# brunnergino/MIDI-VAE

Hardware: AMD Instinct MI355X
Metric: MIDI roll windows/sec (train step) (higher is better)
Workload: dtype bf16

## Files before the change

### midi-vae_amd/csrc/latent.hip

```cpp
#include "common.h"

namespace {

constexpr int LR = 4;
constexpr int LT = 512;
constexpr float CE_EPS = 1e-7f;

template <bool TANH>
__device__ void dense_rows(const float* xs, int ldx, const float* __restrict__ W, int ldw, const float* __restrict__ bias,
                           int K, int N, float* red, float* ys, int ldy, float* yg, int ldg) {
    const int t = threadIdx.x, NV = N / 4;
    for (int c0 = 0; c0 < NV; c0 += LT) {
        const int cur = min(LT, NV - c0), KS = LT / cur, nvl = t % cur, ks = t / cur;
        const int per = ((K + KS - 1) / KS + 3) & ~3;
        if (ks < KS) {
            const int n = (c0 + nvl) * 4;
            f32x4 acc[LR];
#pragma unroll
            for (int r = 0; r < LR; ++r) acc[r] = f32x4{0.f, 0.f, 0.f, 0.f};
            const int k0 = ks * per, k1 = min(K, k0 + per);
            int k = k0;
            for (; k + 16 <= k1; k += 16) {
                f32x4 wv[16];
#pragma unroll
                for (int u = 0; u < 16; ++u) wv[u] = *reinterpret_cast<const f32x4*>(W + (size_t)(k + u) * ldw + n);
#pragma unroll
                for (int r = 0; r < LR; ++r)
#pragma unroll
                    for (int u = 0; u < 16; u += 4) {
                        const f32x4 x = *reinterpret_cast<const f32x4*>(xs + r * ldx + k + u);
                        acc[r] += x[0] * wv[u] + x[1] * wv[u + 1] + x[2] * wv[u + 2] + x[3] * wv[u + 3];
                    }
            }
            for (; k + 4 <= k1; k += 4) {
                f32x4 wv[4];
#pragma unroll
                for (int u = 0; u < 4; ++u) wv[u] = *reinterpret_cast<const f32x4*>(W + (size_t)(k + u) * ldw + n);
#pragma unroll
                for (int r = 0; r < LR; ++r) {
                    const f32x4 x = *reinterpret_cast<const f32x4*>(xs + r * ldx + k);
                    acc[r] += x[0] * wv[0] + x[1] * wv[1] + x[2] * wv[2] + x[3] * wv[3];
                }
            }
            for (; k < k1; ++k) {
                const f32x4 w0 = *reinterpret_cast<const f32x4*>(W + (size_t)k * ldw + n);
#pragma unroll
                for (int r = 0; r < LR; ++r) acc[r] += xs[r * ldx + k] * w0;
            }
#pragma unroll
            for (int r = 0; r < LR; ++r) *reinterpret_cast<f32x4*>(red + ((size_t)(ks * LR + r) * cur + nvl) * 4) = acc[r];
        }
        __syncthreads();
        for (int e = t; e < LR * cur; e += LT) {
            const int r = e / cur, c = e % cur, n = (c0 + c) * 4;
            f32x4 v = {0.f, 0.f, 0.f, 0.f};
            if (bias) v = f32x4{bias[n], bias[n + 1], bias[n + 2], bias[n + 3]};
            for (int s = 0; s < KS; ++s) v += *reinterpret_cast<const f32x4*>(red + ((size_t)(s * LR + r) * cur + c) * 4);
            if (TANH) v = f32x4{tanhf(v[0]), tanhf(v[1]), tanhf(v[2]), tanhf(v[3])};
            if (ys) *reinterpret_cast<f32x4*>(ys + r * ldy + n) = v;
            if (yg) *reinterpret_cast<f32x4*>(yg + (size_t)r * ldg + n) = v;
        }
        __syncthreads();
    }
}

__device__ __forceinline__ int pad4(int n) { return (n + 3) & ~3; }

__global__ __launch_bounds__(LT) void latent_chain_fwd_k(const mvae_latent_chain_fwd_args a) {
    extern __shared__ __attribute__((aligned(16))) float sm[];
    const int H = a.H, Z = a.Z, zin = a.zin, ncH = a.ncat * H, t = threadIdx.x;
    const int r0 = blockIdx.x * LR;
    float* xcat = sm;
    float* h1 = xcat + LR * pad4(ncH);
    float* h2 = h1 + LR * H;
    float* mu = h2 + LR * H;
    float* lv = mu + LR * pad4(Z);
    float* zh = lv + LR * pad4(Z);
    float* red = zh + LR * pad4(zin);
    for (int e = t; e < LR * ncH; e += LT) {
        const int r = e / ncH, c = e % ncH;
        xcat[r * pad4(ncH) + c] = a.cat[(size_t)(r0 + r) * ncH + c];
    }
    __syncthreads();
    const float* h = xcat;
    int ldh = pad4(ncH);
    if (a.w_pack) {
        dense_rows<true>(h, ldh, a.w_pack, H, a.b_pack, ncH, H, red, h1, H, a.pack + (size_t)r0 * H, H);
        h = h1;
        ldh = H;
    }
    if (a.w_extra) {
        dense_rows<true>(h, ldh, a.w_extra, H, a.b_extra, H, H, red, h2, H, a.extra + (size_t)r0 * H, H);
        h = h2;
        ldh = H;
    }
    const int h1w = a.split ? H / 2 : H, h2o = a.split ? h1w : 0, h2w = a.split ? H - h1w : H;
    dense_rows<false>(h, ldh, a.w_mu, Z, a.b_mu, h1w, Z, red, mu, pad4(Z), a.mu + (size_t)r0 * Z, Z);
    dense_rows<false>(h + h2o, ldh, a.w_lv, Z, a.b_lv, h2w, Z, red, lv, pad4(Z), a.logvar + (size_t)r0 * Z, Z);
    {
        const int w = t >> 6, l = t & 63;
        if (w < LR) {
            const int b = r0 + w;
            const float plv = 2.0f * logf(a.prior_std), pvar = a.prior_std * a.prior_std;
            float kl = 0.0f;
            for (int j = l; j < zin; j += 64) {
                float v;
                if (j < Z) {
                    const float m = mu[w * pad4(Z) + j], lg = lv[w * pad4(Z) + j];
                    const float d = m - a.prior_mean;
                    kl += 1.0f + lg - plv - (d * d + expf(lg)) / pvar;
                    v = m + expf(0.5f * lg) * a.eps[(size_t)b * Z + j];
                    a.zh[(size_t)b * zin + j] = v;
                } else {
                    v = a.zh[(size_t)b * zin + j];
                }
                zh[w * pad4(zin) + j] = v;
            }
            kl = wave_sum(kl);
            const bool styled = a.style_target && a.C > 0;
            if (l == 0 && b >= a.B_valid) {
                if (a.kl_rows) a.kl_rows[b] = 0.0f;
                if (a.style_rows && styled) {
                    a.style_rows[(size_t)b * 2] = 0.0f;
                    a.style_rows[(size_t)b * 2 + 1] = 0.0f;
                }
            }
            if (l == 0 && b < a.B_valid) {
                const float klb = a.inv_batch * a.beta * (-0.5f) * kl;
                atomicAdd(a.scalars, klb);
                if (a.kl_rows) a.kl_rows[b] = klb;
                if (styled) {
                    const int C = a.C;
                    const float* zr = zh + w * pad4(zin);
                    float mx = -INFINITY;
                    for (int c = 0; c < C; ++c) mx = fmaxf(mx, zr[c]);
                    float sum = 0.0f;
                    for (int c = 0; c < C; ++c) sum += expf(zr[c] - mx);
                    const int tg = a.style_target[b];
                    float pt = 0.0f, pm = -1.0f;
                    int am = 0;
                    for (int c = 0; c < C; ++c) {
                        const float p = expf(zr[c] - mx) / sum;
                        if (a.style_probs) a.style_probs[(size_t)b * C + c] = p;
                        if (c == tg) pt = p;
                        if (p > pm) { pm = p; am = c; }
                    }
                    const float rw = a.style_row_weight ? a.style_row_weight[b] : a.inv_batch;
                    const float ce = tg < C ? -logf(fminf(fmaxf(pt, CE_EPS), 1.0f - CE_EPS)) : 0.0f;
                    const float hit = am == (tg < C ? tg : 0) ? 1.0f : 0.0f;
                    atomicAdd(a.scalars + 1, rw * ce);
                    atomicAdd(a.scalars + 2, hit);
                    if (a.style_rows) {
                        a.style_rows[(size_t)b * 2] = rw * ce;
                        a.style_rows[(size_t)b * 2 + 1] = hit;
                    }
                }
            }
        }
        __syncthreads();
    }
    if (a.w_init)
        dense_rows<true>(zh, pad4(zin), a.w_init, a.n_init, a.b_init, zin, a.n_init, red, nullptr, 0,
                         a.S + (size_t)r0 * a.n_init, a.n_init);
}

__global__ __launch_bounds__(LT) void latent_chain_bwd_k(const mvae_latent_chain_bwd_args a) {
    extern __shared__ __attribute__((aligned(16))) float sm[];
    const int H = a.H, Z = a.Z, zin = a.zin, ncH = a.ncat * H, NI = a.n_init, t = threadIdx.x;
    const int r0 = blockIdx.x * LR;
    float* ds = sm;
    float* dzh = ds + LR * pad4(NI);
    float* dml = dzh + LR * pad4(zin);
    float* dt = dml + LR * 2 * pad4(Z);
    float* dt2 = dt + LR * H;
    float* dc = dt2 + LR * H;
    float* red = dc + LR * pad4(ncH);
    for (int e = t; e < LR * NI; e += LT) {
        const int r = e / NI, c = e % NI;
        const size_t g = (size_t)(r0 + r) * NI + c;
        const float s = a.S[g], v = a.dS[g] * (1.0f - s * s);
        a.dS[g] = v;
        ds[r * pad4(NI) + c] = v;
    }
    __syncthreads();
    dense_rows<false>(ds, pad4(NI), a.wt_init, zin, nullptr, NI, zin, red, dzh, pad4(zin), nullptr, 0);
    {
        const float pvar = a.prior_std * a.prior_std;
        for (int e = t; e < LR * Z; e += LT) {
            const int r = e / Z, j = e % Z, b = r0 + r;
            float dmu = 0.0f, dlv = 0.0f;
            if (b < a.B_valid) {
                float dz = dzh[r * pad4(zin) + j];
                if (a.style_probs && a.style_target && j < a.C) {
                    const int tg = a.style_target[b];
                    if (tg < a.C) {
                        const float pt = a.style_probs[(size_t)b * a.C + tg];
                        if (pt >= CE_EPS && pt <= 1.0f - CE_EPS) {
                            const float rw = a.style_row_weight ? a.style_row_weight[b] : a.inv_batch;
                            dz += a.style_weight * rw * (a.style_probs[(size_t)b * a.C + j] - (j == tg ? 1.0f : 0.0f));
                        }
                    }
                }
                const float m = a.mu[(size_t)b * Z + j], lg = a.logvar[(size_t)b * Z + j];
                dmu = dz + a.beta * (m - a.prior_mean) / pvar * a.inv_batch;
                dlv = dz * a.eps[(size_t)b * Z + j] * 0.5f * expf(0.5f * lg) +
                      a.beta * (-0.5f) * (1.0f - expf(lg) / pvar) * a.inv_batch;
            }
            a.dmu[(size_t)b * Z + j] = dmu;
            a.dlogvar[(size_t)b * Z + j] = dlv;
            dml[r * 2 * pad4(Z) + j] = dmu;
            dml[r * 2 * pad4(Z) + pad4(Z) + j] = dlv;
        }
        for (int e = t; e < LR * zin; e += LT) a.dzh[(size_t)(r0 + e / zin) * zin + e % zin] = dzh[(e / zin) * pad4(zin) + e % zin];
        __syncthreads();
    }
    const int h1w = a.split ? H / 2 : H, h2w = a.split ? H - h1w : H;
    dense_rows<false>(dml, 2 * pad4(Z), a.wt_mu, h1w, nullptr, Z, h1w, red, dt, H, nullptr, 0);
    if (a.split) {
        dense_rows<false>(dml + pad4(Z), 2 * pad4(Z), a.wt_lv, h2w, nullptr, Z, h2w, red, dt + h1w, H, nullptr, 0);
    } else {
        dense_rows<false>(dml + pad4(Z), 2 * pad4(Z), a.wt_lv, H, nullptr, Z, H, red, dt2, H, nullptr, 0);
        for (int e = t; e < LR * H; e += LT) dt[e] += dt2[e];
        __syncthreads();
    }
    float* cur = dt;
    if (a.wt_extra) {
        for (int e = t; e < LR * H; e += LT) {
            const size_t g = (size_t)(r0 + e / H) * H + e % H;
            const float y = a.extra[g], v = dt[e] * (1.0f - y * y);
            dt[e] = v;
            a.d_extra[g] = v;
        }
        __syncthreads();
        dense_rows<false>(dt, H, a.wt_extra, H, nullptr, H, H, red, dt2, H, nullptr, 0);
        cur = dt2;
    }
    if (a.wt_pack) {
        for (int e = t; e < LR * H; e += LT) {
            const size_t g = (size_t)(r0 + e / H) * H + e % H;
            const float y = a.pack[g], v = cur[e] * (1.0f - y * y);
            cur[e] = v;
            a.d_pack[g] = v;
        }
        __syncthreads();
        dense_rows<false>(cur, H, a.wt_pack, ncH, nullptr, H, ncH, red, nullptr, 0, a.dcat + (size_t)r0 * ncH, ncH);
    } else {
        for (int e = t; e < LR * H; e += LT) a.dcat[(size_t)(r0 + e / H) * H + e % H] = cur[e];
    }
}

size_t fwd_lds(const mvae_latent_chain_fwd_args& a) {
    auto p4 = [](int n) { return (n + 3) & ~3; };
    return sizeof(float) * ((size_t)LR * (p4(a.ncat * a.H) + 2 * a.H + 2 * p4(a.Z) + p4(a.zin)) + (size_t)4 * LR * LT);
}
size_t bwd_lds(const mvae_latent_chain_bwd_args& a) {
    auto p4 = [](int n) { return (n + 3) & ~3; };
    return sizeof(float) * ((size_t)LR * (p4(a.n_init) + p4(a.zin) + 2 * p4(a.Z) + 2 * a.H + p4(a.ncat * a.H)) + (size_t)4 * LR * LT);
}

}

extern "C" int mvae_latent_chain_fwd(const mvae_latent_chain_fwd_args* a, void* stream) {
    if (!a || a->B <= 0 || (a->B % LR) || a->H <= 0 || (a->H % 8) || a->Z <= 0 || (a->Z % 4) || (a->zin % 4) || a->zin < a->Z ||
        a->ncat < 1 || !a->cat || !a->w_mu || !a->w_lv || !a->mu || !a->logvar || !a->eps || !a->zh || !a->scalars)
        return MVAE_E_ARG;
    if ((a->w_pack && !a->pack) || (a->w_extra && !a->extra) || (a->w_init && (!a->S || a->n_init <= 0))) return MVAE_E_ARG;
    if (!a->w_pack && a->ncat != 1) return MVAE_E_ARG;
    if (a->w_init && (a->n_init % 4)) return MVAE_E_ARG;
    if (a->style_target && (a->C <= 0 || a->C > 64 || a->C > a->Z)) return MVAE_E_ARG;
    const size_t lds = fwd_lds(*a);
    if (lds > 160 * 1024) return MVAE_E_UNSUPPORTED;
    return mvae_launch<latent_chain_fwd_k>(dim3(a->B / LR), dim3(LT), lds, reinterpret_cast<hipStream_t>(stream), *a);
}

extern "C" int mvae_latent_chain_bwd(const mvae_latent_chain_bwd_args* a, void* stream) {
    if (!a || a->B <= 0 || (a->B % LR) || a->H <= 0 || (a->H % 8) || a->Z <= 0 || (a->Z % 4) || (a->zin % 4) || a->zin < a->Z ||
        a->ncat < 1 || a->n_init <= 0 || (a->n_init % 4) || !a->S || !a->dS || !a->wt_init || !a->wt_mu || !a->wt_lv || !a->mu ||
        !a->logvar || !a->eps || !a->dzh || !a->dmu || !a->dlogvar || !a->dcat)
        return MVAE_E_ARG;
    if ((a->wt_pack && (!a->pack || !a->d_pack)) || (a->wt_extra && (!a->extra || !a->d_extra))) return MVAE_E_ARG;
    if (!a->wt_pack && a->ncat != 1) return MVAE_E_ARG;
    const size_t lds = bwd_lds(*a);
    if (lds > 160 * 1024) return MVAE_E_UNSUPPORTED;
    return mvae_launch<latent_chain_bwd_k>(dim3(a->B / LR), dim3(LT), lds, reinterpret_cast<hipStream_t>(stream), *a);
}
```

Before: 40180.

## Double-buffer weight loads and prefetch next stage's first tile across dense stages

Rewrites dense_rows as a software-pipelined loop with two 16-row register buffers, loading the next weight tile while FMAs run on the current one. The first tile of the following layer is prefetched before the reduction barrier, so the chain of dense layers in the latent forward and backward kernels overlaps weight fetch latency with compute and with reductions. Tail rows are handled by clamped loads in place of the scalar remainder loops. This costs extra registers (two 16-entry f32x4 buffers), which may reduce occupancy or cause spills, and adds more control logic per iteration.

```diff
diff --git a/midi-vae_amd/csrc/latent.hip b/midi-vae_amd/csrc/latent.hip
--- a/midi-vae_amd/csrc/latent.hip
+++ b/midi-vae_amd/csrc/latent.hip
@@ -6,59 +6,110 @@
 constexpr int LT = 512;
 constexpr float CE_EPS = 1e-7f;
 
+struct Stage {
+    const float* W;
+    int ldw, K, N;
+};
+
+struct Slice {
+    int cur, KS, nvl, ks, n, k0, k1;
+};
+
+__device__ __forceinline__ Slice slice_of(const Stage& s, int c0) {
+    const int t = threadIdx.x, NV = s.N / 4;
+    Slice q;
+    q.cur = min(LT, NV - c0);
+    q.KS = LT / q.cur;
+    q.nvl = t % q.cur;
+    q.ks = t / q.cur;
+    const int per = ((s.K + q.KS - 1) / q.KS + 3) & ~3;
+    q.n = (c0 + q.nvl) * 4;
+    q.k0 = q.ks < q.KS ? q.ks * per : 0;
+    q.k1 = q.ks < q.KS ? min(s.K, q.k0 + per) : 0;
+    return q;
+}
+
+__device__ __forceinline__ void load_round(f32x4 (&b)[16], const float* __restrict__ W, int ldw, int K, int row0, int n) {
+    if (row0 + 16 <= K) {
+#pragma unroll
+        for (int u = 0; u < 16; ++u) b[u] = *reinterpret_cast<const f32x4*>(W + (size_t)(row0 + u) * ldw + n);
+    } else {
+#pragma unroll
+        for (int u = 0; u < 16; ++u) b[u] = *reinterpret_cast<const f32x4*>(W + (size_t)min(row0 + u, K - 1) * ldw + n);
+    }
+}
+
+__device__ __forceinline__ void prefetch_round(f32x4 (&b)[16], const Stage& s, int c0) {
+    if (!s.W) return;
+    const Slice q = slice_of(s, c0);
+    if (q.k0 < q.k1) load_round(b, s.W, s.ldw, s.K, q.k0, q.n);
+}
+
+__device__ __forceinline__ void fma_round(f32x4 (&acc)[LR], const f32x4 (&b)[16], const float* xs, int ldx, int k, int k1) {
+    if (k + 16 <= k1) {
+#pragma unroll
+        for (int r = 0; r < LR; ++r)
+#pragma unroll
+            for (int u = 0; u < 16; u += 4) {
+                const f32x4 x = *reinterpret_cast<const f32x4*>(xs + r * ldx + k + u);
+                acc[r] += x[0] * b[u] + x[1] * b[u + 1] + x[2] * b[u + 2] + x[3] * b[u + 3];
+            }
+    } else {
+#pragma unroll
+        for (int u = 0; u < 12; u += 4)
+            if (k + u + 4 <= k1) {
+#pragma unroll
+                for (int r = 0; r < LR; ++r) {
+                    const f32x4 x = *reinterpret_cast<const f32x4*>(xs + r * ldx + k + u);
+                    acc[r] += x[0] * b[u] + x[1] * b[u + 1] + x[2] * b[u + 2] + x[3] * b[u + 3];
+                }
+            }
+    }
+}
+
 template <bool TANH>
-__device__ void dense_rows(const float* xs, int ldx, const float* __restrict__ W, int ldw, const float* __restrict__ bias,
-                           int K, int N, float* red, float* ys, int ldy, float* yg, int ldg) {
-    const int t = threadIdx.x, NV = N / 4;
+__device__ __forceinline__ void dense_rows(f32x4 (&pf)[16], const float* xs, int ldx, const Stage& st, const float* __restrict__ bias,
+                                           const Stage& nx, float* red, float* ys, int ldy, float* yg, int ldg) {
+    const int t = threadIdx.x, NV = st.N / 4;
+    const float* __restrict__ W = st.W;
+    const int ldw = st.ldw, K = st.K;
     for (int c0 = 0; c0 < NV; c0 += LT) {
-        const int cur = min(LT, NV - c0), KS = LT / cur, nvl = t % cur, ks = t / cur;
-        const int per = ((K + KS - 1) / KS + 3) & ~3;
+        const Slice sl = slice_of(st, c0);
+        const int cur = sl.cur, KS = sl.KS, nvl = sl.nvl, ks = sl.ks, n = sl.n, k1 = sl.k1;
+        const bool last = c0 + LT >= NV;
+        const Stage& after = last ? nx : st;
+        Slice a = {};
+        if (after.W) a = slice_of(after, last ? 0 : c0 + LT);
+        const float* aW = after.W && a.k0 < a.k1 ? after.W : nullptr;
+        f32x4 q[16], acc[LR];
+#pragma unroll
+        for (int r = 0; r < LR; ++r) acc[r] = f32x4{0.f, 0.f, 0.f, 0.f};
+        for (int k = sl.k0;;) {
+            const bool more1 = k + 16 < k1;
+            if (more1) load_round(q, W, ldw, K, k + 16, n);
+            fma_round(acc, pf, xs, ldx, k, k1);
+            k += 16;
+            const bool more2 = k + 16 < k1;
+            const float* lW = more2 ? W : aW;
+            if (lW) load_round(pf, lW, more2 ? ldw : after.ldw, more2 ? K : after.K, more2 ? k + 16 : a.k0, more2 ? n : a.n);
+            if (!more1) break;
+            fma_round(acc, q, xs, ldx, k, k1);
+            if (!more2) break;
+            k += 16;
+        }
         if (ks < KS) {
-            const int n = (c0 + nvl) * 4;
-            f32x4 acc[LR];
-#pragma unroll
-            for (int r = 0; r < LR; ++r) acc[r] = f32x4{0.f, 0.f, 0.f, 0.f};
-            const int k0 = ks * per, k1 = min(K, k0 + per);
-            int k = k0;
-            for (; k + 16 <= k1; k += 16) {
-                f32x4 wv[16];
-#pragma unroll
-                for (int u = 0; u < 16; ++u) wv[u] = *reinterpret_cast<const f32x4*>(W + (size_t)(k + u) * ldw + n);
-#pragma unroll
-                for (int r = 0; r < LR; ++r)
-#pragma unroll
-                    for (int u = 0; u < 16; u += 4) {
-                        const f32x4 x = *reinterpret_cast<const f32x4*>(xs + r * ldx + k + u);
-                        acc[r] += x[0] * wv[u] + x[1] * wv[u + 1] + x[2] * wv[u + 2] + x[3] * wv[u + 3];
-                    }
-            }
-            for (; k + 4 <= k1; k += 4) {
-                f32x4 wv[4];
-#pragma unroll
-                for (int u = 0; u < 4; ++u) wv[u] = *reinterpret_cast<const f32x4*>(W + (size_t)(k + u) * ldw + n);
-#pragma unroll
-                for (int r = 0; r < LR; ++r) {
-                    const f32x4 x = *reinterpret_cast<const f32x4*>(xs + r * ldx + k);
-                    acc[r] += x[0] * wv[0] + x[1] * wv[1] + x[2] * wv[2] + x[3] * wv[3];
-                }
-            }
-            for (; k < k1; ++k) {
-                const f32x4 w0 = *reinterpret_cast<const f32x4*>(W + (size_t)k * ldw + n);
-#pragma unroll
-                for (int r = 0; r < LR; ++r) acc[r] += xs[r * ldx + k] * w0;
-            }
 #pragma unroll
             for (int r = 0; r < LR; ++r) *reinterpret_cast<f32x4*>(red + ((size_t)(ks * LR + r) * cur + nvl) * 4) = acc[r];
         }
         __syncthreads();
         for (int e = t; e < LR * cur; e += LT) {
-            const int r = e / cur, c = e % cur, n = (c0 + c) * 4;
+            const int r = e / cur, c = e % cur, nc = (c0 + c) * 4;
             f32x4 v = {0.f, 0.f, 0.f, 0.f};
-            if (bias) v = f32x4{bias[n], bias[n + 1], bias[n + 2], bias[n + 3]};
+            if (bias) v = f32x4{bias[nc], bias[nc + 1], bias[nc + 2], bias[nc + 3]};
             for (int s = 0; s < KS; ++s) v += *reinterpret_cast<const f32x4*>(red + ((size_t)(s * LR + r) * cur + c) * 4);
             if (TANH) v = f32x4{tanhf(v[0]), tanhf(v[1]), tanhf(v[2]), tanhf(v[3])};
-            if (ys) *reinterpret_cast<f32x4*>(ys + r * ldy + n) = v;
-            if (yg) *reinterpret_cast<f32x4*>(yg + (size_t)r * ldg + n) = v;
+            if (ys) *reinterpret_cast<f32x4*>(ys + r * ldy + nc) = v;
+            if (yg) *reinterpret_cast<f32x4*>(yg + (size_t)r * ldg + nc) = v;
         }
         __syncthreads();
     }
@@ -77,6 +128,12 @@
     float* lv = mu + LR * pad4(Z);
     float* zh = lv + LR * pad4(Z);
     float* red = zh + LR * pad4(zin);
+    const int h1w = a.split ? H / 2 : H, h2o = a.split ? h1w : 0, h2w = a.split ? H - h1w : H;
+    const Stage s_pack = {a.w_pack, H, ncH, H}, s_extra = {a.w_extra, H, H, H}, s_mu = {a.w_mu, Z, h1w, Z}, s_lv = {a.w_lv, Z, h2w, Z},
+                s_init = {a.w_init, a.n_init, zin, a.n_init}, s_none = {nullptr, 0, 0, 0};
+    const Stage& s_tail = a.w_extra ? s_extra : s_mu;
+    f32x4 pf[16];
+    prefetch_round(pf, a.w_pack ? s_pack : s_tail, 0);
     for (int e = t; e < LR * ncH; e += LT) {
         const int r = e / ncH, c = e % ncH;
         xcat[r * pad4(ncH) + c] = a.cat[(size_t)(r0 + r) * ncH + c];
@@ -85,18 +142,17 @@
     const float* h = xcat;
     int ldh = pad4(ncH);
     if (a.w_pack) {
-        dense_rows<true>(h, ldh, a.w_pack, H, a.b_pack, ncH, H, red, h1, H, a.pack + (size_t)r0 * H, H);
+        dense_rows<true>(pf, h, ldh, s_pack, a.b_pack, s_tail, red, h1, H, a.pack + (size_t)r0 * H, H);
         h = h1;
         ldh = H;
     }
     if (a.w_extra) {
-        dense_rows<true>(h, ldh, a.w_extra, H, a.b_extra, H, H, red, h2, H, a.extra + (size_t)r0 * H, H);
+        dense_rows<true>(pf, h, ldh, s_extra, a.b_extra, s_mu, red, h2, H, a.extra + (size_t)r0 * H, H);
         h = h2;
         ldh = H;
     }
-    const int h1w = a.split ? H / 2 : H, h2o = a.split ? h1w : 0, h2w = a.split ? H - h1w : H;
-    dense_rows<false>(h, ldh, a.w_mu, Z, a.b_mu, h1w, Z, red, mu, pad4(Z), a.mu + (size_t)r0 * Z, Z);
-    dense_rows<false>(h + h2o, ldh, a.w_lv, Z, a.b_lv, h2w, Z, red, lv, pad4(Z), a.logvar + (size_t)r0 * Z, Z);
+    dense_rows<false>(pf, h, ldh, s_mu, a.b_mu, s_lv, red, mu, pad4(Z), a.mu + (size_t)r0 * Z, Z);
+    dense_rows<false>(pf, h + h2o, ldh, s_lv, a.b_lv, s_init, red, lv, pad4(Z), a.logvar + (size_t)r0 * Z, Z);
     {
         const int w = t >> 6, l = t & 63;
         if (w < LR) {
@@ -160,8 +216,7 @@
         __syncthreads();
     }
     if (a.w_init)
-        dense_rows<true>(zh, pad4(zin), a.w_init, a.n_init, a.b_init, zin, a.n_init, red, nullptr, 0,
-                         a.S + (size_t)r0 * a.n_init, a.n_init);
+        dense_rows<true>(pf, zh, pad4(zin), s_init, a.b_init, s_none, red, nullptr, 0, a.S + (size_t)r0 * a.n_init, a.n_init);
 }
 
 __global__ __launch_bounds__(LT) void latent_chain_bwd_k(const mvae_latent_chain_bwd_args a) {
@@ -175,6 +230,11 @@
     float* dt2 = dt + LR * H;
     float* dc = dt2 + LR * H;
     float* red = dc + LR * pad4(ncH);
+    const int h1w = a.split ? H / 2 : H, h2w = a.split ? H - h1w : H;
+    const Stage s_init = {a.wt_init, zin, NI, zin}, s_mu = {a.wt_mu, h1w, Z, h1w}, s_lv = {a.wt_lv, h2w, Z, h2w},
+                s_extra = {a.wt_extra, H, H, H}, s_pack = {a.wt_pack, ncH, H, ncH};
+    f32x4 pf[16];
+    prefetch_round(pf, s_init, 0);
     for (int e = t; e < LR * NI; e += LT) {
         const int r = e / NI, c = e % NI;
         const size_t g = (size_t)(r0 + r) * NI + c;
@@ -183,7 +243,7 @@
         ds[r * pad4(NI) + c] = v;
     }
     __syncthreads();
-    dense_rows<false>(ds, pad4(NI), a.wt_init, zin, nullptr, NI, zin, red, dzh, pad4(zin), nullptr, 0);
+    dense_rows<false>(pf, ds, pad4(NI), s_init, nullptr, s_mu, red, dzh, pad4(zin), nullptr, 0);
     {
         const float pvar = a.prior_std * a.prior_std;
         for (int e = t; e < LR * Z; e += LT) {
@@ -214,12 +274,12 @@
         for (int e = t; e < LR * zin; e += LT) a.dzh[(size_t)(r0 + e / zin) * zin + e % zin] = dzh[(e / zin) * pad4(zin) + e % zin];
         __syncthreads();
     }
-    const int h1w = a.split ? H / 2 : H, h2w = a.split ? H - h1w : H;
-    dense_rows<false>(dml, 2 * pad4(Z), a.wt_mu, h1w, nullptr, Z, h1w, red, dt, H, nullptr, 0);
+    const Stage& s_tail = a.wt_extra ? s_extra : s_pack;
+    dense_rows<false>(pf, dml, 2 * pad4(Z), s_mu, nullptr, s_lv, red, dt, H, nullptr, 0);
     if (a.split) {
-        dense_rows<false>(dml + pad4(Z), 2 * pad4(Z), a.wt_lv, h2w, nullptr, Z, h2w, red, dt + h1w, H, nullptr, 0);
+        dense_rows<false>(pf, dml + pad4(Z), 2 * pad4(Z), s_lv, nullptr, s_tail, red, dt + h1w, H, nullptr, 0);
     } else {
-        dense_rows<false>(dml + pad4(Z), 2 * pad4(Z), a.wt_lv, H, nullptr, Z, H, red, dt2, H, nullptr, 0);
+        dense_rows<false>(pf, dml + pad4(Z), 2 * pad4(Z), s_lv, nullptr, s_tail, red, dt2, H, nullptr, 0);
         for (int e = t; e < LR * H; e += LT) dt[e] += dt2[e];
         __syncthreads();
     }
@@ -232,7 +292,7 @@
             a.d_extra[g] = v;
         }
         __syncthreads();
-        dense_rows<false>(dt, H, a.wt_extra, H, nullptr, H, H, red, dt2, H, nullptr, 0);
+        dense_rows<false>(pf, dt, H, s_extra, nullptr, s_pack, red, dt2, H, nullptr, 0);
         cur = dt2;
     }
     if (a.wt_pack) {
@@ -243,7 +303,7 @@
             a.d_pack[g] = v;
         }
         __syncthreads();
-        dense_rows<false>(cur, H, a.wt_pack, ncH, nullptr, H, ncH, red, nullptr, 0, a.dcat + (size_t)r0 * ncH, ncH);
+        dense_rows<false>(pf, cur, H, s_pack, nullptr, Stage{nullptr, 0, 0, 0}, red, nullptr, 0, a.dcat + (size_t)r0 * ncH, ncH);
     } else {
         for (int e = t; e < LR * H; e += LT) a.dcat[(size_t)(r0 + e / H) * H + e % H] = cur[e];
     }
```

Measured after the change: 40470 (median of 6 runs). About the same (+0.7%).
